# dusk-network/plonk

Measured on AMD Instinct MI355X. Metric: prove() wall-clock (ms) at 2^20 gates, lower is better.
Workload: dtype u32 limbs (Fr 256-bit / Fp 384-bit Montgomery)

## Files before the change

__graft_entry__.py:

```python
from __future__ import annotations

import concurrent.futures as cf
import os
import shutil
import subprocess
import sys

ROOT = os.path.dirname(os.path.abspath(__file__))
CSRC = os.path.join(ROOT, "plonk_amd", "csrc")
LIBDIR = os.path.join(ROOT, "plonk_amd", "lib")
OBJDIR = os.path.join(ROOT, "build", "obj")
LIB = os.path.join(LIBDIR, "libplonk_hip.so")
HIP_SOURCES = ["ntt.hip", "msm.hip", "msm_sort.hip", "capi.hip", "poly.hip", "prover.hip", "serial.hip", "comm.hip", "verify.hip", "diagnose.hip", "kzg.hip", "composer.hip", "msm_points.hip", "pairing.hip", "kzg_domain.hip"]
MSM_LARGE_BITS = os.environ.get("PLONK_BUILD_MSM_LARGE_BITS", "19")
MSM_MEDIUM = os.environ.get("PLONK_BUILD_MSM_MEDIUM", "") == "1"
HIP_VARIANTS = [("msm.hip", "nbl" + MSM_LARGE_BITS, ["-DPLONK_MSM_NB_BITS=" + MSM_LARGE_BITS]),
                ("msm_sort.hip", "nbl" + MSM_LARGE_BITS, ["-DPLONK_MSM_NB_BITS=" + MSM_LARGE_BITS])]
if MSM_MEDIUM:
    HIP_VARIANTS += [("msm.hip", "nbm17", ["-DPLONK_MSM_NB_BITS=17", "-DPLONK_MSM_WITH_MEDIUM"]),
                     ("msm_sort.hip", "nbm17", ["-DPLONK_MSM_NB_BITS=17", "-DPLONK_MSM_WITH_MEDIUM"])]
    HIP_FLAGS_EXTRA = ["-DPLONK_MSM_WITH_MEDIUM"]
else:
    HIP_FLAGS_EXTRA = []
HIPCC = shutil.which("hipcc") or "/opt/rocm/bin/hipcc"
# ... 65 lines not shown
        os.makedirs(os.path.dirname(DEV_ARITH_LIB), exist_ok=True)
        os.makedirs(OBJDIR, exist_ok=True)

        def compile_group(group: str) -> str:
            obj = os.path.join(OBJDIR, "dev_arith." + group + ".o")
            if _newer(obj, deps):
                subprocess.check_call([HIPCC, *HIP_FLAGS, "-DARITH_GROUP=ARITH_FAMILIES_" + group, "-c", src, "-o", obj])
            return obj

        with cf.ThreadPoolExecutor(max_workers=len(DEV_ARITH_GROUPS)) as ex:
            objs = list(ex.map(compile_group, DEV_ARITH_GROUPS))
        subprocess.check_call([HIPCC, "--offload-arch=gfx950", "-shared", "-fPIC", *objs, "-o", DEV_ARITH_LIB])
    if verbose:
        print(f"[build] {DEV_ARITH_LIB}")
    return DEV_ARITH_LIB


DEV_POLY_LIB = os.path.join(ROOT, "tests", "_build", "libdev_poly.so")


def build_dev_poly(verbose: bool = True) -> str:
    src = os.path.join(ROOT, "tests", "csrc", "dev_poly.hip")
    if not os.path.exists(src):
        return DEV_POLY_LIB
    if _newer(DEV_POLY_LIB, [src, LIB] + _headers()):
        os.makedirs(os.path.dirname(DEV_POLY_LIB), exist_ok=True)
        subprocess.check_call([HIPCC, *HIP_FLAGS, "-I" + CSRC, "-shared", src, "-o", DEV_POLY_LIB,
                               "-L" + LIBDIR, "-lplonk_hip", "-Wl,-rpath,$ORIGIN/../../plonk_amd/lib"])
    if verbose:
        print(f"[build] {DEV_POLY_LIB}")
    return DEV_POLY_LIB


DEV_MSM_SORT_LIB = os.path.join(ROOT, "tests", "_build", "libdev_msm_sort.so")


def build_dev_msm_sort(verbose: bool = True) -> str:
    src = os.path.join(ROOT, "tests", "csrc", "dev_msm_sort.hip")
    if not os.path.exists(src):
        return DEV_MSM_SORT_LIB
    if _newer(DEV_MSM_SORT_LIB, [src, LIB] + _headers()):
        os.makedirs(os.path.dirname(DEV_MSM_SORT_LIB), exist_ok=True)
        subprocess.check_call([HIPCC, *HIP_FLAGS, "-I" + CSRC, "-shared", src, "-o", DEV_MSM_SORT_LIB,
                               "-L" + LIBDIR, "-lplonk_hip", "-Wl,-rpath,$ORIGIN/../../plonk_amd/lib"])
    if verbose:
        print(f"[build] {DEV_MSM_SORT_LIB}")
    return DEV_MSM_SORT_LIB


DEV_KZG_DOMAIN_LIB = os.path.join(ROOT, "tests", "_build", "libdev_kzg_domain.so")


def build_dev_kzg_domain(verbose: bool = True) -> str:
    src = os.path.join(ROOT, "tests", "csrc", "dev_kzg_domain.hip")
    if not os.path.exists(src):
        return DEV_KZG_DOMAIN_LIB
    if _newer(DEV_KZG_DOMAIN_LIB, [src, LIB] + _headers()):
        os.makedirs(os.path.dirname(DEV_KZG_DOMAIN_LIB), exist_ok=True)
        subprocess.check_call([HIPCC, *HIP_FLAGS, "-I" + CSRC, "-shared", src, "-o", DEV_KZG_DOMAIN_LIB,
                               "-L" + LIBDIR, "-lplonk_hip", "-Wl,-rpath,$ORIGIN/../../plonk_amd/lib"])
    if verbose:
        print(f"[build] {DEV_KZG_DOMAIN_LIB}")
    return DEV_KZG_DOMAIN_LIB


def build() -> None:
    with cf.ThreadPoolExecutor(max_workers=1) as side:
        dev_arith = side.submit(build_dev_arith)
        build_hip()
        build_dev_poly()
        build_dev_msm_sort()
        build_dev_kzg_domain()
        build_oracle()
        build_fake_rccl()
        dev_arith.result()
    sys.path.insert(0, ROOT)
    import plonk_amd
    plonk_amd.load_library()


def smoke() -> None:
    sys.path.insert(0, ROOT)
    import random

    import plonk_amd
    from oracle import bls12_381 as E
    from oracle.fft import EvaluationDomain

    ctx = plonk_amd.Context(0)
    rnd = random.Random(7)
    L = 12
    coeffs = [rnd.randrange(E.Q) for _ in range((1 << 9) + 3)]
    got = ctx.ntt(coeffs, L, inverse=False, coset=True)
    assert got == EvaluationDomain(1 << L).coset_fft(coeffs), "NTT mismatch vs oracle"
    pts = [E.g1_mul(E.G1_GEN, rnd.randrange(1, E.Q)) for _ in range(64)]
    sc = [rnd.randrange(E.Q) for _ in range(64)]
    ctx.srs_load(pts)
    assert ctx.msm(sc) == E.msm_pippenger(pts, sc), "MSM mismatch vs oracle"
    print("smoke ok: NTT(2^12 coset) and MSM(64) bit-exact vs oracle")


if __name__ == "__main__":
    build()
# ... 1 lines not shown
```

plonk_amd/csrc/poly.hip:

```cpp
#include <cstdlib>

#include "plonk_internal.hpp"
#include "fr29.cuh"
#include "fp_safegcd.cuh"
#include "poly.hpp"

namespace plonk {

__device__ __forceinline__ Fr ldf(const Fr* p) {
  const uint4* q = reinterpret_cast<const uint4*>(p);
  uint4 a = q[0], b = q[1];
  Fr r;
  r.l[0] = a.x; r.l[1] = a.y; r.l[2] = a.z; r.l[3] = a.w;
  r.l[4] = b.x; r.l[5] = b.y; r.l[6] = b.z; r.l[7] = b.w;
  return r;
}
__device__ __forceinline__ void stf(Fr* p, const Fr& v) {
  uint4* q = reinterpret_cast<uint4*>(p);
  q[0] = make_uint4(v.l[0], v.l[1], v.l[2], v.l[3]);
  q[1] = make_uint4(v.l[4], v.l[5], v.l[6], v.l[7]);
}
__device__ __forceinline__ Fr small(uint32_t v, const Fr& one) {
  Fr acc = Fr::zero();
  Fr p = one;
  for (uint32_t b = v; b; b >>= 1) {
    if (b & 1) acc = acc + p;
    p = p.dbl();
  }
  return acc;
}

__global__ void fill_zero_kernel(Fr* p, uint64_t n) {
  const uint64_t i = (uint64_t)blockIdx.x * blockDim.x + threadIdx.x;
// ... 394 lines not shown
  HIP_TRY(hipGetLastError());
  return PLONK_OK;
}
int scan_prefix_product_apply(Ctx* c, Fr* data, uint64_t n, const Fr* totals, const Fr& carry_twiddle) {
  const uint32_t nb = scan_prefix_blocks(n);
  PScanArgs a{};
  a.one_t = tw_of(Fr::one());
  a.one_r = tw_plain(Fr::one());
  a.carry_t = tw_plain(carry_twiddle);
  a.has_carry = 1;
  pscan_launch_apply(c, nb, data, n, totals, a);
  HIP_TRY(hipGetLastError());
  return PLONK_OK;
}
int scan_suffix_sum(Ctx* c, Fr* data, uint64_t n, Fr* totals) { return scan_inplace<false, true>(c, data, n, totals); }

struct PermConst {
  Tw conv;
  Tw gamma_t;
  Tw bk_t[4];
  Tw b32_t;
  Tw one_t;
};
__device__ __forceinline__ Fr29 ld_slot(const void* base, uint64_t idx) {
  const uint4* q = reinterpret_cast<const uint4*>(reinterpret_cast<const Fr29Slot*>(base) + idx);
  const uint4 a = q[0], b = q[1];
  const uint32_t c = reinterpret_cast<const Fr29Slot*>(base)[idx].w[8];
  Fr29 r;
  r.l[0] = a.x; r.l[1] = a.y; r.l[2] = a.z; r.l[3] = a.w;
  r.l[4] = b.x; r.l[5] = b.y; r.l[6] = b.z; r.l[7] = b.w;
  r.l[8] = c;
  return r;
}
__global__ void __launch_bounds__(128) perm_terms_kernel(PermArgs a, PermConst k) {
  const uint64_t j0 = (uint64_t)blockIdx.x * blockDim.x + threadIdx.x;
  if (j0 >= a.count) return;
  const uint64_t i = a.first + j0;
  if (i == 0) {
    const Fr one = tw29(k.one_t).to_fr();
    stf(a.num, one);
    stf(a.den, one);
    return;
  }
  const uint64_t r = i - 1;
  Fr29 root = ld_slot(a.tw_lo29, r & ((1ull << a.lobits) - 1));
  if (a.use_hi) root = Fr29::mul(root, ld_slot(a.tw_hi29, r >> a.lobits));
  const Fr29 conv = tw29(k.conv), gamma_t = tw29(k.gamma_t), b32 = tw29(k.b32_t);
  Fr29 num, den;
#pragma unroll
  for (int j = 0; j < 4; ++j) {
    const Fr29 wg = Fr29::add_csub(Fr29::mul(ld29_(a.wires[j] + r), conv), gamma_t);
    const Fr29 nf = Fr29::add_csub(wg, Fr29::mul(root, tw29(k.bk_t[j])));
    const Fr29 df = Fr29::add_csub(wg, Fr29::mul(ld29_(a.sigma[j] + r), b32));
    num = j ? Fr29::mul(num, nf) : nf;
    den = j ? Fr29::mul(den, df) : df;
  }
  stf(a.num + i, num.to_fr());
  stf(a.den + i, den.to_fr());
}
__global__ void mul_arrays_kernel(Fr* __restrict__ a, const Fr* __restrict__ b, uint64_t n, int* zero_flag) {
  const uint64_t i = (uint64_t)blockIdx.x * blockDim.x + threadIdx.x;
  if (i >= n) return;
  const Fr y = ldf(b + i);
  if (zero_flag && y.is_zero()) *zero_flag = 1;
  stf(a + i, Fr29::mul(ld29_(a + i), Fr29::from_fr(y)).to_fr());
}

__device__ __forceinline__ Fr delta4(const Fr& f, const Fr& one) {
  const Fr two = one.dbl();
  return f * (f - one) * (f - two) * (f - two - one);
}

__device__ __forceinline__ Fr29 ld29(const Fr* p) { return Fr29::from_fr(ldf(p)); }
__device__ __forceinline__ Fr29 c29(const uint32_t (&v)[9]) {
  Fr29 r;
#pragma unroll
  for (int i = 0; i < 9; ++i) r.l[i] = v[i];
  return r;
}

struct WidgetConst {
  Tw conv, one_r, c1, c3, c9, c18, c81, c83, ed;
  Tw rg[4];
  Tw lg[5];
  Tw fx[4];
  Tw vr[3];
};
template <bool WIDGETS>
__global__ void __launch_bounds__(128, WIDGETS ? 2 : 4) quotient_kernel(QuotientArgs q, WidgetConst wc) {
  const uint64_t i = (uint64_t)blockIdx.x * blockDim.x + threadIdx.x;
  if (i >= q.n8) return;
// ... 223 lines not shown
  uint32_t nbits;
  uint64_t zero_at;
};
template <int E>
__global__ void __launch_bounds__(256) mul_powers_kernel(const Fr* __restrict__ src, Fr* __restrict__ dst, uint64_t n,
                                                         MulPowArgs a, uint64_t src_off, uint64_t exp_off) {
  const uint64_t g = (uint64_t)blockIdx.x * blockDim.x + threadIdx.x;
  if (g == 0 && a.zero_at != ~0ull) stf(dst + a.zero_at, Fr::zero());
  const uint64_t wave = g >> 6, lane = g & 63;
  const uint64_t first = wave * (64 * E) + lane;
  if (first >= n) return;
  const Fr29 add = Fr29::from_fr(a.addend);
  const uint64_t e = first + exp_off;
  Fr29 p = tw29(a.one_t);
  bool started = false;
#pragma unroll 1
  for (uint32_t b = 0; b < a.nbits; ++b) {
    if ((e >> b) & 1) {
      const Fr29 w = tw29(a.pw[b]);
      p = started ? Fr29::mul(p, w) : w;
      started = true;
    }
  }
  const Fr29 step = tw29(a.pw[6]);
#pragma unroll 1
  for (int k = 0; k < E; ++k) {
    const uint64_t i = first + 64ull * k;
    if (i >= n) break;
    stf(dst + i, Fr29::mul(Fr29::add_csub(ld29_(src + i + src_off), add), p).to_fr());
    if (E > 1) p = Fr29::mul(p, step);
  }
}

__global__ void fold_kernel(const Fr* __restrict__ src, Fr* __restrict__ dst, uint64_t n, uint32_t extra, Fr c) {
  const uint64_t i = (uint64_t)blockIdx.x * blockDim.x + threadIdx.x;
  if (i >= n) return;
  Fr v = ldf(src + i);
  if (i < extra) v = v + c * ldf(src + n + i);
  stf(dst + i, v);
}

__global__ void shard_pack_kernel(ShardPackArgs a) {
  const uint64_t i = (uint64_t)blockIdx.x * blockDim.x + threadIdx.x;
  const uint32_t k = blockIdx.y, peer = blockIdx.z;
  if (i >= a.stride) return;
  const Fr* F = a.F[k];
  Fr v = Fr::zero();
  if (i < a.per) {
    const uint64_t idx = (uint64_t)peer * a.per + i;
    if (idx < a.n) v = ldf(F + idx);
  } else {
    v = ldf(F + (i - a.per));
  }
  stf(a.send + ((uint64_t)peer * a.cpr + k) * a.stride + i, v);
}

__global__ void __launch_bounds__(128) shard_combine_kernel(ShardCombineArgs a) {
  const uint64_t i = (uint64_t)blockIdx.x * blockDim.x + threadIdx.x;
  if (i >= a.cnt + 8) return;
  const bool extra = i >= a.cnt;
  const uint64_t off = extra ? a.per + (i - a.cnt) : i;
  Fr F[8];
  for (uint32_t j = 0; j < a.Q; ++j)
    F[j] = ldf(a.recv + ((uint64_t)(j % a.W) * a.cpr + j / a.W) * a.stride + off);
  auto dft = [&](uint32_t i1) {
    Fr acc = Fr::zero();
// ... 68 lines not shown
  hipLaunchKernelGGL(gather_wires_kernel, grid, dim3(256), 0, c->stream, idx_dev, values, wires, constraints, n);
  HIP_TRY(hipGetLastError());
  return PLONK_OK;
}
int poly_scatter_pi(Ctx* c, Fr* dense, const uint64_t* idx, const Fr* val, uint64_t count) {
  if (!count) return PLONK_OK;
  hipLaunchKernelGGL(scatter_pi_kernel, grid1(count, 256), dim3(256), 0, c->stream, dense, idx, val, count);
  HIP_TRY(hipGetLastError());
  return PLONK_OK;
}
int poly_batch_inverse(Ctx* c, Fr* v, uint64_t n, bool twiddle_form) {
  static const BatchInvArgs a = [] {
    BatchInvArgs r;
    r.one_t = tw_of(Fr::one());
    r.one_r = tw_plain(Fr::one());
    r.conv = tw_of(Fr::from_u64(32));
    return r;
  }();
  const int cfg_env = c->cfg.bi_cfg;
  const int cfg = cfg_env >= 0 && cfg_env <= 3 ? cfg_env : (n <= (1ull << 17) ? 1 : 0);
#define BI_LAUNCH(T, E)                                                                                                              \
  do {                                                                                                                               \
    if (twiddle_form) hipLaunchKernelGGL((batch_inverse_kernel<true, T, E>), grid1(n, T * E), dim3(T), 0, c->stream, v, n, a);         \
    else hipLaunchKernelGGL((batch_inverse_kernel<false, T, E>), grid1(n, T * E), dim3(T), 0, c->stream, v, n, a);                     \
  } while (0)
  if (cfg == 1) BI_LAUNCH(64, 4);
  else if (cfg == 2) BI_LAUNCH(64, 16);
  else if (cfg == 3) BI_LAUNCH(128, 8);
  else BI_LAUNCH(256, 16);
#undef BI_LAUNCH
  HIP_TRY(hipGetLastError());
  return PLONK_OK;
}
int poly_perm_terms(Ctx* c, const PermArgs& a) {
  PermConst k;
  k.conv = tw_of(Fr::from_u64(32));
  k.gamma_t = tw_of(a.gamma);
  for (int j = 0; j < 4; ++j) k.bk_t[j] = tw_of(a.beta * a.ks[j]);
  k.b32_t = tw_of(a.beta * Fr::from_u64(32));
  k.one_t = tw_of(Fr::one());
  PermArgs r = a;
  if (r.count == 0) { r.first = 0; r.count = a.n; }
  if (r.first + r.count > a.n) return (plonk::set_last_error("invalid argument", __func__, __FILE__, __LINE__), PLONK_ERR_ARG);
  hipLaunchKernelGGL(perm_terms_kernel, grid1(r.count, 128), dim3(128), 0, c->stream, r, k);
  HIP_TRY(hipGetLastError());
  return PLONK_OK;
}
int poly_mul_arrays(Ctx* c, Fr* a, const Fr* b, uint64_t n, int* zero_flag) {
  hipLaunchKernelGGL(mul_arrays_kernel, grid1(n, 256), dim3(256), 0, c->stream, a, b, n, zero_flag);
  HIP_TRY(hipGetLastError());
  return PLONK_OK;
}
int poly_quotient(Ctx* c, const QuotientArgs& q) {
  prof_begin(c, 3);
  WidgetConst wc{};
  if (q.has[QS_RANGE] | q.has[QS_LOGIC] | q.has[QS_FIXED] | q.has[QS_VAR]) {
    wc.conv = tw_of(Fr::from_u64(32));
    wc.one_r = tw_plain(Fr::one());
    wc.c1 = tw_of(Fr::one()); wc.c3 = tw_of(Fr::from_u64(3)); wc.c9 = tw_of(Fr::from_u64(9));
    wc.c18 = tw_of(Fr::from_u64(18)); wc.c81 = tw_of(Fr::from_u64(81)); wc.c83 = tw_of(Fr::from_u64(83));
    wc.ed = tw_of(q.edwards_d);
    Fr k = q.range_ch.sqr(), w = q.range_ch;
    for (int j = 0; j < 4; ++j) { wc.rg[j] = tw_of(w); w = w * k; }
    k = q.logic_ch.sqr();
    const Fr lk[5] = {k.sqr() * k, Fr::one(), k, k.sqr(), k.sqr().sqr()};
    for (int j = 0; j < 5; ++j) wc.lg[j] = tw_of(lk[j] * q.logic_ch);
    k = q.fixed_ch.sqr(); w = q.fixed_ch;
    for (int j = 0; j < 4; ++j) { wc.fx[j] = tw_of(w); w = w * k; }
    k = q.var_ch.sqr(); w = q.var_ch;
    for (int j = 0; j < 3; ++j) { wc.vr[j] = tw_of(w); w = w * k; }
    hipLaunchKernelGGL(quotient_kernel<true>, grid1(q.n8, 128), dim3(128), 0, c->stream, q, wc);
  } else {
    hipLaunchKernelGGL(quotient_kernel<false>, grid1(q.n8, 128), dim3(128), 0, c->stream, q, wc);
// ... 48 lines not shown
  EvalArgsD d;
  Fr pts[EV_POINTS];
  int npts = 0;
  for (int k = 0; k < count; ++k) {
    d.items[k].poly = a.items[k].poly;
    d.items[k].len = a.items[k].len;
    int w = 0;
    while (w < npts && !(pts[w] == a.items[k].x)) ++w;
    if (w == npts) {
      if (npts == EV_POINTS) return (plonk::set_last_error("invalid argument", "poly_eval: more than 2 distinct points", __FILE__, __LINE__), PLONK_ERR_ARG);
      pts[npts++] = a.items[k].x;
      Fr29 p = Fr29::twiddle_from_fr(a.items[k].x);
      for (int b = 0; b < EV_PW; ++b) {
        for (int i = 0; i < 9; ++i) d.pw[w][b].w[i] = p.l[i];
        p = Fr29::mul(p, p);
      }
    }
    d.items[k].point = (uint32_t)w;
  }
  d.partial = a.partial;
  d.max_blocks = a.max_blocks;
  int levels = 0;
  while (levels < 8 && (1u << levels) < nb) ++levels;
  if (le == 2) {
    hipLaunchKernelGGL(eval_kernel<2>, dim3(nb, count), dim3(EV_T), 0, c->stream, d);
    hipLaunchKernelGGL(eval_final_kernel<2>, dim3(count), dim3(EV_T), 0, c->stream, d, nb, levels, out_dev);
  } else {
    hipLaunchKernelGGL(eval_kernel<4>, dim3(nb, count), dim3(EV_T), 0, c->stream, d);
    hipLaunchKernelGGL(eval_final_kernel<4>, dim3(count), dim3(EV_T), 0, c->stream, d, nb, levels, out_dev);
  }
  HIP_TRY(hipGetLastError());
  return PLONK_OK;
}
int poly_lincomb(Ctx* c, const LinCombArgs& a) {
  LinCombArgsD d;
  for (int k = 0; k < a.count; ++k) {
    d.t[k].p = a.t[k].p;
    d.t[k].len = a.t[k].len;
    d.t[k].st = tw_of(a.t[k].s);
  }
  d.count = a.count;
  d.len = a.len;
  d.constant = a.constant;
  d.out = a.out;
  hipLaunchKernelGGL(lincomb_kernel, grid1(a.len, 256), dim3(256), 0, c->stream, d);
  HIP_TRY(hipGetLastError());
  return PLONK_OK;
}
static void launch_mul_powers(Ctx* c, const Fr* src, Fr* dst, uint64_t n, const Fr& x, uint64_t src_off, uint64_t exp_off,
                              const Fr& addend = Fr::zero(), uint64_t zero_at = ~0ull) {
  if (!n) {
    if (zero_at != ~0ull) (void)poly_fill_zero(c, dst + zero_at, 1);
    return;
  }
  MulPowArgs a;
  const uint64_t emax = n - 1 + exp_off;
  uint32_t nbits = 7;
  while (nbits < MP_BITS && (emax >> nbits)) ++nbits;
  Fr29 p = Fr29::twiddle_from_fr(x);
  for (uint32_t b = 0; b < nbits; ++b) {
    for (int i = 0; i < 9; ++i) a.pw[b].w[i] = p.l[i];
    p = Fr29::mul(p, p);
  }
  a.one_t = tw_of(Fr::one());
  a.addend = addend;
  a.nbits = nbits;
  a.zero_at = zero_at;
  if (n <= (1ull << 17)) hipLaunchKernelGGL(mul_powers_kernel<1>, grid1(n, 256), dim3(256), 0, c->stream, src, dst, n, a, src_off, exp_off);
  else if (n <= (1ull << 19)) hipLaunchKernelGGL(mul_powers_kernel<4>, grid1((n + 3) / 4 + 64, 256), dim3(256), 0, c->stream, src, dst, n, a, src_off, exp_off);
  else hipLaunchKernelGGL(mul_powers_kernel<16>, grid1((n + 15) / 16 + 64, 256), dim3(256), 0, c->stream, src, dst, n, a, src_off, exp_off);
}
int poly_ruffini(Ctx* c, const Fr* src, Fr* dst, uint64_t len, const Fr& z, const Fr& zinv, Fr* scratch, Fr* totals) {
  launch_mul_powers(c, src, scratch, len, z, 0, 0);
  int rc = scan_suffix_sum(c, scratch, len, totals);
  if (rc) return rc;
  launch_mul_powers(c, scratch, dst, len - 1, zinv, 1, 1, Fr::zero(), len - 1);
  HIP_TRY(hipGetLastError());
  return PLONK_OK;
}

__device__ __forceinline__ void st_slot(void* base, uint64_t idx, const Fr29& v) {
  uint32_t* w = reinterpret_cast<Fr29Slot*>(base)[idx].w;
#pragma unroll
  for (int i = 0; i < 9; ++i) w[i] = v.l[i];
  w[9] = 0; w[10] = 0; w[11] = 0;
}
__global__ void __launch_bounds__(256) kzg_powers_kernel(void* __restrict__ tab, uint32_t count, Tw xt, Tw one_t) {
  const uint32_t i = blockIdx.x * blockDim.x + threadIdx.x;
  if (i >= count) return;
  st_slot(tab, i, pow_tw(tw29(xt), i, tw29(one_t)));
}
__global__ void __launch_bounds__(256) power_array_kernel(Fr* __restrict__ out, uint64_t n, Tw xt, Tw one_t) {
  const uint64_t i = (uint64_t)blockIdx.x * blockDim.x + threadIdx.x;
  if (i >= n) return;
  stf(out + i, Fr29::mul(Fr29::from_fr(Fr::one()), pow_tw(tw29(xt), i, tw29(one_t))).to_fr());
}
__global__ void __launch_bounds__(256) kzg_trim_kernel(KzgDesc* __restrict__ desc) {
  __shared__ unsigned long long best;
  const Fr* p = desc[blockIdx.x].p;
  uint64_t hi = desc[blockIdx.x].len;
  while (hi) {
    if (!threadIdx.x) best = 0;
    __syncthreads();
    const uint64_t lo = hi > 256 ? hi - 256 : 0, idx = lo + threadIdx.x;
    if (idx < hi && !ldf(p + idx).is_zero()) atomicMax(&best, (unsigned long long)(idx + 1));
    __syncthreads();
    const uint64_t b = best;
    __syncthreads();
    if (b) { hi = b; break; }
// ... 135 lines not shown
```

plonk_amd/csrc/poly.hpp:

```cpp
#pragma once
#include "plonk_internal.hpp"

namespace plonk {

enum { QS_M = 0, QS_L, QS_R, QS_O, QS_F, QS_C, QS_ARITH, QS_RANGE, QS_LOGIC, QS_FIXED, QS_VAR, QS_COUNT };

struct BlindArgs {
  int count;
  Fr b[3];
};
struct SplitArgs {
  Fr b[3];
  uint64_t len4;
};
struct PermArgs {
  uint64_t n;
  uint64_t first = 0, count = 0;
  const Fr* wires[4];
  const Fr* sigma[4];
  Fr beta, gamma;
  Fr ks[4];
  const void* tw_lo29;
  const void* tw_hi29;
  uint32_t lobits;
// ... 107 lines not shown

void prof_begin(Ctx* c, int slot);
void prof_end(Ctx* c, int slot);
void prof_host_add(Ctx* c, int slot, double ms);

int poly_fill_zero(Ctx* c, Fr* p, uint64_t n);
int poly_blind(Ctx* c, Fr* coeffs, uint64_t n, const BlindArgs& a);
int poly_split_t(Ctx* c, Fr* t, uint64_t n, uint64_t np, Fr* out, const SplitArgs& a);
int poly_trimmed_len(Ctx* c, const Fr* p, uint64_t n, unsigned long long* out_dev);
int poly_scatter_pi(Ctx* c, Fr* dense, const uint64_t* idx, const Fr* val, uint64_t count);
int poly_sigma_evals(Ctx* c, const uint32_t* map_dev, const Fr* roots, Fr* out, uint64_t n, uint64_t stride, const SigmaArgs& a);
int poly_gather_wires(Ctx* c, const uint32_t* idx_dev, const Fr* values, Fr* wires, uint64_t constraints, uint64_t n);
int poly_batch_inverse(Ctx* c, Fr* v, uint64_t n, bool twiddle_form = false);
int poly_perm_terms(Ctx* c, const PermArgs& a);
int poly_mul_arrays(Ctx* c, Fr* a, const Fr* b, uint64_t n, int* zero_flag);
int poly_quotient(Ctx* c, const QuotientArgs& q);
int poly_dealias(Ctx* c, Fr* t, uint64_t nq, const Fr low[7], const Fr& g_inv);
int poly_l1(Ctx* c, const Fr* linear, Fr* l1, uint64_t n8, const L1Args& a);
int poly_scale_array(Ctx* c, Fr* v, uint64_t n, const Fr& s);
int poly_from_mont(Ctx* c, const Fr* src, Fr* dst, uint64_t n);
void quotient_const(const Fr& c, int shift, uint32_t out[9]);
void quotient_data(const Fr& c, uint32_t out[9]);
int poly_eval(Ctx* c, EvalArgs& a, int count, uint64_t max_len, Fr* out_dev);
int poly_lincomb(Ctx* c, const LinCombArgs& a);
int poly_ruffini(Ctx* c, const Fr* src, Fr* dst, uint64_t len, const Fr& z, const Fr& zinv, Fr* scratch, Fr* totals);
static constexpr int SCAN_T = 256;
static constexpr int SCAN_MAXPER = 64;
static constexpr uint64_t SCAN_TOTALS = SCAN_T * SCAN_MAXPER + 1;
int scan_prefix_product(Ctx* c, Fr* data, uint64_t n, Fr* totals);
uint32_t scan_prefix_blocks(uint64_t n);
int scan_prefix_product_local(Ctx* c, Fr* data, uint64_t n, Fr* totals);
int scan_prefix_product_apply(Ctx* c, Fr* data, uint64_t n, const Fr* totals, const Fr& carry_twiddle);
int scan_suffix_sum(Ctx* c, Fr* data, uint64_t n, Fr* totals);

}
```

plonk_amd/csrc/prover.hip:

```cpp
#include <cstdlib>
#include <cstring>
#include <random>
#include <string>
#include <vector>

#include "poly.hpp"
#include "transcript.hpp"
#include <chrono>

#include "hostg1.hpp"
#include "finish_pool.hpp"
#include "widgets.hpp"
#include "permutation.hpp"
#include "diagnose.hpp"
#include "composer.hpp"

static_assert(plonk::DQ_M == plonk::QS_M && plonk::DQ_ARITH == plonk::QS_ARITH && plonk::DQ_VAR == plonk::QS_VAR &&
              plonk::DQ_COUNT == plonk::QS_COUNT, "diagnose_core.hpp selector ids");
static_assert(plonk::WQS_RANGE == plonk::QS_RANGE && plonk::WQS_LOGIC == plonk::QS_LOGIC && plonk::WQS_FIXED == plonk::QS_FIXED &&
              plonk::WQS_VAR == plonk::QS_VAR && plonk::WQS_COUNT == plonk::QS_COUNT, "widgets.hpp selector ids");

namespace plonk {

struct Prover {
// ... 990 lines not shown
      AccMark mark(c, (side_defer && k0 + kc == 4) ? p->ev_acc : nullptr);
      PTRY(msm_group(p, sc, ms, 4, 0, p->lag_table, p->lag_n, tl, sp, 1, k0, kc));
    }
    PTRY(msm_group(p, sc, ms, 4, 0, p->lag_table, p->lag_n, tl, sp, 2));
  } else {
    p->last_wire_launches = 1;
    AccMark mark(c, side_defer ? p->ev_acc : nullptr);
    const uint64_t ms[4] = {n + 2, n + 2, n + 2, n + 2};
    if (lag) {
      const Fr* sc[4] = {wires_dev, wires_dev + n, wires_dev + 2 * n, wires_dev + 3 * n};
      const Fr* tl[4] = {p->wscal, p->wscal + 2, p->wscal + 4, p->wscal + 6};
      const uint64_t sp[4] = {n, n, n, n};
      PTRY(msm_group(p, sc, ms, 4, 0, p->lag_table, p->lag_n, tl, sp));
    } else {
      const Fr* sc[4] = {p->wpoly, p->wpoly + np, p->wpoly + 2 * np, p->wpoly + 3 * np};
      PTRY(msm_group(p, sc, ms, 4, 0));
    }
  }
  if (side_defer) {
    SideScopeAfter side(c, p->ev_acc);
    PTRY(side_round1());
  }
  PTRY(absorb_commitments(p, tr, 0, 4, comm));

  Challenges ch;
  ch.beta = tr.challenge_scalar("beta");
  tr.append_scalar("beta", ch.beta);
  ch.gamma = tr.challenge_scalar("gamma");
  {
    prof_begin(c, 4);
    const PermArgs pa = perm_args(p, wires_dev, ch, tbn);
    gap.launching();
    HIP_TRY(hipMemsetAsync(p->flag_dev, 0, sizeof(int), c->stream));
    PTRY(poly_perm_terms(c, pa));
    PTRY(poly_batch_inverse(c, pa.den, n, true));
    PTRY(poly_mul_arrays(c, pa.num, pa.den, n, p->flag_dev));
    PTRY(scan_prefix_product(c, pa.num, n, p->totals));
    if (!z_from_evals) PTRY(blind_z(p, pa.num, bl, p->tmp8));
    prof_end(c, 4);
  }
  auto side_round2 = [&]() -> int {
    if (z_from_evals) {
      PTRY(blind_z(p, p->scratch, bl, p->tmp8b));
      HIP_TRY(hipMemcpyAsync(p->low_host + 28, p->zpoly, 7 * sizeof(Fr), hipMemcpyDeviceToHost, c->stream));
      HIP_TRY(hipEventRecord(p->ev_zlow, c->stream));
    }
    PTRY(ntt_device(c, p->zpoly, p->cos, p->tmp8b, L + p->lq, false, true, n + 3));
    HIP_TRY(hipEventRecord(p->ev_side, c->side_stream));
    return PLONK_OK;
  };
  if (z_from_evals) {
    HIP_TRY(hipMemcpyAsync(p->wscal + 8, bl + 8, 3 * sizeof(Fr), hipMemcpyHostToDevice, c->stream));
  } else {
    HIP_TRY(hipMemcpyAsync(p->low_host + 28, p->zpoly, 7 * sizeof(Fr), hipMemcpyDeviceToHost, c->stream));
    HIP_TRY(hipEventRecord(p->ev_zlow, c->stream));
  }
  if (!side_defer_z) {
    SideScope side(c, p->ev_ready);
    PTRY(side_round2());
  }
  {
    AccMark mark(c, side_defer_z ? p->ev_acc : nullptr);
    if (z_from_evals) {
      const Fr* sc[1] = {p->scratch};
      const Fr* tl[1] = {p->wscal + 8};
      const uint64_t ms[1] = {n + 3}, sp[1] = {n};
      PTRY(msm_group(p, sc, ms, 1, 4, p->lag_table, p->lag_n, tl, sp));
    } else {
      PTRY(msm_to(p, p->zpoly, n + 3, 4));
    }
// ... 53 lines not shown
    const uint64_t ms[4] = {n + 1, n + 1, n + 1, t4_len};
    PTRY(msm_group(p, sc, ms, 4, 5));
  }
  PTRY(absorb_commitments(p, tr, 5, 4, comm));
  if (*p->flag_host) return (plonk::set_last_error("invalid argument", __func__, __FILE__, __LINE__), PLONK_ERR_ARG);

  const Fr z_ch = tr.challenge_scalar("z_challenge");
  const Fr zw = z_ch * omega;
  Evals ev;
  {
    EvalArgs ea;
    const uint64_t max_len = eval_items(p, z_ch, zw, 0, np, &ea);
    gap.launching();
    PTRY(poly_eval(c, ea, 15, max_len, p->evout));
    HIP_TRY(hipMemcpyAsync(p->ev_host, p->evout, 15 * sizeof(Fr), hipMemcpyDeviceToHost, c->stream));
    const auto t_before = HostGap::clock::now();
    HIP_TRY(hipStreamSynchronize(c->stream));
    gap.synced(t_before);
    ev = unpack_evals(p->ev_host);
  }
  append_evaluations(tr, ev);

  const Fr v = tr.challenge_scalar("v_challenge");
  Opening op;
  PTRY(opening_point(p, z_ch, zw, &op));
  const Fr v_w = tr.challenge_scalar("v_w_challenge");
  {
    gap.launching();
    SideScope side(c, p->ev_ready);
    LinCombArgs la;
    wzw_terms(p, v_w, 0, np, &la);
    la.len = np - 1;
    la.constant = Fr::zero();
    la.out = p->tmp8;
    PTRY(poly_lincomb(c, la));
    PTRY(poly_ruffini(c, p->tmp8, p->wit2, np - 1, zw, op.inv_z * p->omega_inv, p->scratch + np, p->totals2));
    HIP_TRY(hipEventRecord(p->ev_side, c->side_stream));
  }
  opening_scalars(p, ev, ch, z_ch, v, pi_idx, pi_val, pi_count, &op);
  {
    LinCombArgs la;
    numerator_terms(p, ev, ch, op, t4, t4_len, 0, np, &la);
    la.len = np - 1;
    la.constant = op.pi_eval;
    la.out = p->agg;
    gap.launching();
    PTRY(poly_lincomb(c, la));
  }
  PTRY(poly_ruffini(c, p->agg, p->wit, np - 1, z_ch, op.inv_z, p->scratch, p->totals));
  HIP_TRY(hipMemcpyAsync(p->evout + 15, p->scratch, sizeof(Fr), hipMemcpyDeviceToDevice, c->stream));
  HIP_TRY(hipMemcpyAsync(p->ev_host + 15, p->evout + 15, sizeof(Fr), hipMemcpyDeviceToHost, c->stream));
  HIP_TRY(hipStreamWaitEvent(c->main_stream, p->ev_side, 0));
  {
    const Fr* sc[2] = {p->wit, p->wit2};
    const uint64_t ms[2] = {np - 2, np - 2};
    PTRY(msm_group(p, sc, ms, 2, 9));
  }
  PTRY(fetch_commitments(p, 9, 2, comm + 9));
  if (!quotient_identity_holds(p->ev_host[15], ev, ch.alpha, ch.beta, ch.gamma, op.l1_z, op.vp)) return PLONK_ERR_UNSAT;

  write_proof(proof, comm, ev);
  return PLONK_OK;
}

static int prover_prove_sharded(Prover* p, const Fr* wires_dev, const uint64_t* pi_idx, const Fr* pi_val, uint64_t pi_count,
                                const Fr* bl, uint8_t proof[1008]) {
  Ctx* c = p->c;
  if (p->srs_gen != c->srs_gen) return (set_last_error("prover is bound to an SRS that was replaced on its context", __func__, __FILE__, __LINE__), PLONK_ERR_STATE);
  const uint64_t n = p->n, np = p->np, qn = p->qn;
  const uint32_t L = p->logn, W = (uint32_t)p->world, cpr = p->cpr, Q = p->Q;
  const uint64_t lo = p->lo, hi = p->hi;
  NttTables* tbn;
  PTRY(ntt_tables(c, L, false, &tbn));
  const Fr omega = p->omega;

  Transcript tr((const uint8_t*)p->label.data(), p->label.size());
  seed_transcript(tr, p, pi_val, pi_count);
  HostGap gap{c};
  GapScope gap_scope(&gap);

  uint8_t comm[11][48];
  const bool lag = p->lag_on;
// ... 869 lines not shown
```

Before: 31.30.

## Fuse permutation grand product and lincomb+Ruffini into blockwise scan kernels

```diff
diff --git a/__graft_entry__.py b/__graft_entry__.py
--- a/__graft_entry__.py
+++ b/__graft_entry__.py
@@ -121,6 +121,22 @@
     return DEV_POLY_LIB
 
 
+DEV_POLY_FUSED_LIB = os.path.join(ROOT, "tests", "_build", "libdev_poly_fused.so")
+
+
+def build_dev_poly_fused(verbose: bool = True) -> str:
+    src = os.path.join(ROOT, "tests", "csrc", "dev_poly_fused.hip")
+    if not os.path.exists(src):
+        return DEV_POLY_FUSED_LIB
+    if _newer(DEV_POLY_FUSED_LIB, [src, LIB] + _headers()):
+        os.makedirs(os.path.dirname(DEV_POLY_FUSED_LIB), exist_ok=True)
+        subprocess.check_call([HIPCC, *HIP_FLAGS, "-I" + CSRC, "-shared", src, "-o", DEV_POLY_FUSED_LIB,
+                               "-L" + LIBDIR, "-lplonk_hip", "-Wl,-rpath,$ORIGIN/../../plonk_amd/lib"])
+    if verbose:
+        print(f"[build] {DEV_POLY_FUSED_LIB}")
+    return DEV_POLY_FUSED_LIB
+
+
 DEV_MSM_SORT_LIB = os.path.join(ROOT, "tests", "_build", "libdev_msm_sort.so")
 
 
@@ -158,6 +174,7 @@
         dev_arith = side.submit(build_dev_arith)
         build_hip()
         build_dev_poly()
+        build_dev_poly_fused()
         build_dev_msm_sort()
         build_dev_kzg_domain()
         build_oracle()
diff --git a/plonk_amd/csrc/poly.hip b/plonk_amd/csrc/poly.hip
--- a/plonk_amd/csrc/poly.hip
+++ b/plonk_amd/csrc/poly.hip
@@ -1,4 +1,5 @@
 #include <cstdlib>
+#include <type_traits>
 
 #include "plonk_internal.hpp"
 #include "fr29.cuh"
@@ -459,6 +460,22 @@
   r.l[8] = c;
   return r;
 }
+__device__ __forceinline__ void perm_row(const PermArgs& a, const PermConst& k, uint64_t r, Fr29* num_out, Fr29* den_out) {
+  Fr29 root = ld_slot(a.tw_lo29, r & ((1ull << a.lobits) - 1));
+  if (a.use_hi) root = Fr29::mul(root, ld_slot(a.tw_hi29, r >> a.lobits));
+  const Fr29 conv = tw29(k.conv), gamma_t = tw29(k.gamma_t), b32 = tw29(k.b32_t);
+  Fr29 num, den;
+#pragma unroll
+  for (int j = 0; j < 4; ++j) {
+    const Fr29 wg = Fr29::add_csub(Fr29::mul(ld29_(a.wires[j] + r), conv), gamma_t);
+    const Fr29 nf = Fr29::add_csub(wg, Fr29::mul(root, tw29(k.bk_t[j])));
+    const Fr29 df = Fr29::add_csub(wg, Fr29::mul(ld29_(a.sigma[j] + r), b32));
+    num = j ? Fr29::mul(num, nf) : nf;
+    den = j ? Fr29::mul(den, df) : df;
+  }
+  *num_out = num;
+  *den_out = den;
+}
 __global__ void __launch_bounds__(128) perm_terms_kernel(PermArgs a, PermConst k) {
   const uint64_t j0 = (uint64_t)blockIdx.x * blockDim.x + threadIdx.x;
   if (j0 >= a.count) return;
@@ -469,21 +486,130 @@
     stf(a.den, one);
     return;
   }
-  const uint64_t r = i - 1;
-  Fr29 root = ld_slot(a.tw_lo29, r & ((1ull << a.lobits) - 1));
-  if (a.use_hi) root = Fr29::mul(root, ld_slot(a.tw_hi29, r >> a.lobits));
-  const Fr29 conv = tw29(k.conv), gamma_t = tw29(k.gamma_t), b32 = tw29(k.b32_t);
   Fr29 num, den;
-#pragma unroll
-  for (int j = 0; j < 4; ++j) {
-    const Fr29 wg = Fr29::add_csub(Fr29::mul(ld29_(a.wires[j] + r), conv), gamma_t);
-    const Fr29 nf = Fr29::add_csub(wg, Fr29::mul(root, tw29(k.bk_t[j])));
-    const Fr29 df = Fr29::add_csub(wg, Fr29::mul(ld29_(a.sigma[j] + r), b32));
-    num = j ? Fr29::mul(num, nf) : nf;
-    den = j ? Fr29::mul(den, df) : df;
-  }
+  perm_row(a, k, i - 1, &num, &den);
   stf(a.num + i, num.to_fr());
   stf(a.den + i, den.to_fr());
+}
+
+__device__ __forceinline__ bool is_zero29(const Fr29& x) {
+  const Fr29 c = x.csub_q();
+  uint32_t any = 0;
+#pragma unroll
+  for (int i = 0; i < 9; ++i) any |= c.l[i];
+  return any == 0;
+}
+__device__ __forceinline__ void ps_lanes_both(Fr29& p, Fr29& s, uint32_t (*shp)[SCAN_T], uint32_t (*shs)[SCAN_T], int t,
+                                              const Fr29& one_t, Fr29* ptot, Fr29* stot) {
+  for (int d = 1; d < SCAN_T; d <<= 1) {
+    ps_put(shp, t, p);
+    ps_put(shs, t, s);
+    __syncthreads();
+    if (t >= d) p = Fr29::mul(ps_get(shp, t - d), p);
+    if (t + d < SCAN_T) s = Fr29::mul(ps_get(shs, t + d), s);
+    __syncthreads();
+  }
+  ps_put(shp, t, p);
+  ps_put(shs, t, s);
+  __syncthreads();
+  p = t ? ps_get(shp, t - 1) : one_t;
+  s = (t + 1 < SCAN_T) ? ps_get(shs, t + 1) : one_t;
+  *ptot = ps_get(shp, SCAN_T - 1);
+  *stot = ps_get(shs, 0);
+}
+template <int I, int N, class F>
+__device__ __forceinline__ void unrolled(F&& f) {
+  if constexpr (I < N) {
+    f(std::integral_constant<int, I>{});
+    unrolled<I + 1, N>(f);
+  }
+}
+template <int E>
+__global__ void __launch_bounds__(SCAN_T) gp_block_kernel(PermArgs a, PermConst k, Fr* __restrict__ totals, uint32_t nb, int* flag) {
+  __shared__ uint32_t shp[9][SCAN_T], shs[9][SCAN_T];
+  const int t = threadIdx.x;
+  const uint64_t base = (uint64_t)blockIdx.x * (SCAN_T * E) + (uint64_t)t * E;
+  const Fr29 one_t = tw29(k.one_t);
+  Fr29 v[E], d[E];
+  Fr29 accn = one_t, accd = one_t;
+  unrolled<0, E>([&](auto ec) {
+    constexpr int e = decltype(ec)::value;
+    const uint64_t i = base + e;
+    d[e] = one_t;
+    if (i > 0 && i < a.n) {
+      Fr29 num, den;
+      perm_row(a, k, i - 1, &num, &den);
+      if (is_zero29(den)) *flag = 1;
+      else d[e] = den;
+      accn = Fr29::mul(accn, num);
+      accd = Fr29::mul(accd, d[e]);
+    }
+    v[e] = accn;
+  });
+  Fr29 ntot, dtot;
+  ps_lanes_both(accn, accd, shp, shs, t, one_t, &ntot, &dtot);
+  if (t == 0) {
+    stf(totals + blockIdx.x, ntot.to_fr());
+    stf(totals + nb + blockIdx.x, dtot.to_fr());
+  }
+  unrolled<0, E>([&](auto ec) {
+    constexpr int e = E - 1 - decltype(ec)::value;
+    const uint64_t i = base + e;
+    if (i < a.n) {
+      stf(a.num + i, Fr29::mul(accn, v[e]).to_fr());
+      stf(a.den + i, accd.to_fr());
+    }
+    accd = Fr29::mul(accd, d[e]);
+  });
+}
+__global__ void __launch_bounds__(SCAN_T) gp_totals_kernel(Fr* __restrict__ totals, uint32_t nb, uint32_t per, PScanArgs a) {
+  __shared__ uint32_t shp[9][SCAN_T], shs[9][SCAN_T], shinv[9];
+  const int t = threadIdx.x;
+  Fr* const tn = totals;
+  const Fr* const td = totals + nb;
+  const Fr29 one_t = tw29(a.one_t);
+  Fr29 accn = one_t, accd = one_t;
+  for (uint32_t j = 0; j < per; ++j) {
+    const uint32_t i = t * per + j;
+    if (i < nb) {
+      accn = Fr29::mul(accn, ld29_(tn + i));
+      accd = Fr29::mul(accd, ld29_(td + i));
+    }
+  }
+  Fr29 ntot, dtot;
+  ps_lanes_both(accn, accd, shp, shs, t, one_t, &ntot, &dtot);
+  if (t == 0) {
+    const Fr29 r = fr29_inv_gcd_tw(dtot);
+#pragma unroll
+    for (int i = 0; i < 9; ++i) shinv[i] = r.l[i];
+  }
+  __syncthreads();
+  Fr29 inv;
+#pragma unroll
+  for (int i = 0; i < 9; ++i) inv.l[i] = shinv[i];
+  for (uint32_t j = 0; j < per; ++j) {
+    const uint32_t i = t * per + j;
+    if (i < nb) {
+      const Fr29 x = ld29_(tn + i);
+      stf(tn + i, accn.to_fr());
+      accn = Fr29::mul(accn, x);
+    }
+  }
+  accd = Fr29::mul(Fr29::mul(accd, inv), tw29(a.one_r));
+  for (uint32_t j = per; j-- > 0;) {
+    const uint32_t i = t * per + j;
+    if (i < nb) {
+      stf(tn + i, Fr29::mul(ld29_(tn + i), accd).to_fr());
+      accd = Fr29::mul(accd, ld29_(td + i));
+    }
+  }
+}
+__global__ void __launch_bounds__(256) gp_apply_kernel(const Fr* a, const Fr* b, Fr* z, uint64_t n, const Fr* __restrict__ totals,
+                                                       uint32_t block_log) {
+  const uint64_t i = (uint64_t)blockIdx.x * blockDim.x + threadIdx.x;
+  if (i >= n) return;
+  const Fr29 c = ld29_(totals + (i >> block_log));
+  stf(z + i, Fr29::mul(Fr29::mul(ld29_(a + i), ld29_(b + i)), c).to_fr());
 }
 __global__ void mul_arrays_kernel(Fr* __restrict__ a, const Fr* __restrict__ b, uint64_t n, int* zero_flag) {
   const uint64_t i = (uint64_t)blockIdx.x * blockDim.x + threadIdx.x;
@@ -773,6 +899,111 @@
   }
 }
 
+static inline int lrscan_e(uint64_t len) { return len <= (1ull << 17) ? 2 : 4; }
+template <int E>
+__global__ void __launch_bounds__(SCAN_T) lincomb_ruffini_block_kernel(LinCombArgsD a, MulPowArgs m, Fr* __restrict__ scratch,
+                                                                       Fr* __restrict__ totals, uint32_t nb) {
+  __shared__ Fr sh[SCAN_T];
+  const int t = threadIdx.x;
+  const uint64_t base = (uint64_t)blockIdx.x * (SCAN_T * E) + (uint64_t)t * E;
+  Fr29 p = tw29(m.one_t);
+  if (base < a.len) {
+    bool started = false;
+#pragma unroll 1
+    for (uint32_t b = 0; b < m.nbits; ++b) {
+      if ((base >> b) & 1) {
+        const Fr29 w = tw29(m.pw[b]);
+        p = started ? Fr29::mul(p, w) : w;
+        started = true;
+      }
+    }
+  }
+  const Fr29 step = tw29(m.pw[0]);
+  Fr29 c[E];
+  unrolled<0, E>([&](auto ec) {
+    constexpr int e = decltype(ec)::value;
+    c[e] = (base + e == 0) ? Fr29::from_fr(a.constant) : Fr29::zero();
+  });
+  for (int k = 0; k < a.count; ++k) {
+    const Fr* const tp = a.t[k].p;
+    const uint64_t tl = a.t[k].len;
+    const Fr29 st = tw29(a.t[k].st);
+    unrolled<0, E>([&](auto ec) {
+      constexpr int e = decltype(ec)::value;
+      if (base + e < tl) c[e] = Fr29::add_csub(c[e], Fr29::mul(ld29_(tp + base + e), st));
+    });
+  }
+  Fr v[E];
+  unrolled<0, E>([&](auto ec) {
+    constexpr int e = decltype(ec)::value;
+    v[e] = Fr::zero();
+    if (base + e < a.len) {
+      v[e] = Fr29::mul(c[e], p).to_fr();
+      p = Fr29::mul(p, step);
+    }
+  });
+  Fr acc = Fr::zero();
+  unrolled<0, E>([&](auto ec) {
+    constexpr int e = E - 1 - decltype(ec)::value;
+    acc = acc + v[e];
+    v[e] = acc;
+  });
+  sh[t] = acc;
+  __syncthreads();
+  for (int d = 1; d < SCAN_T; d <<= 1) {
+    Fr x = Fr::zero();
+    const bool take = t + d < SCAN_T;
+    if (take) x = sh[t + d];
+    __syncthreads();
+    if (take) sh[t] = sh[t] + x;
+    __syncthreads();
+  }
+  const Fr excl = (t + 1 < SCAN_T) ? sh[t + 1] : Fr::zero();
+  if (t == 0) stf(totals + (nb - 1 - blockIdx.x), sh[0]);
+  unrolled<0, E>([&](auto ec) {
+    constexpr int e = decltype(ec)::value;
+    if (base + e < a.len) stf(scratch + base + e, excl + v[e]);
+  });
+}
+template <int E>
+__global__ void __launch_bounds__(256) ruffini_apply_kernel(Fr* __restrict__ scratch, Fr* __restrict__ dst, uint64_t n, MulPowArgs a,
+                                                            const Fr* __restrict__ totals, uint32_t nb, uint32_t block_log) {
+  const uint64_t g = (uint64_t)blockIdx.x * blockDim.x + threadIdx.x;
+  if (g == 0) {
+    stf(dst + n, Fr::zero());
+    if (nb > 1) stf(scratch, ldf(scratch) + ldf(totals + nb - 2));
+  }
+  const uint64_t wave = g >> 6, lane = g & 63;
+  const uint64_t first = wave * (64 * E) + lane;
+  if (first >= n) return;
+  const uint64_t e = first + 1;
+  Fr29 p = tw29(a.one_t);
+  bool started = false;
+#pragma unroll 1
+  for (uint32_t b = 0; b < a.nbits; ++b) {
+    if ((e >> b) & 1) {
+      const Fr29 w = tw29(a.pw[b]);
+      p = started ? Fr29::mul(p, w) : w;
+      started = true;
+    }
+  }
+  const Fr29 step = tw29(a.pw[6]);
+  uint64_t cur = ~0ull;
+  Fr off = Fr::zero();
+#pragma unroll 1
+  for (int k = 0; k < E; ++k) {
+    const uint64_t i = first + 64ull * k;
+    if (i >= n) break;
+    const uint64_t b = (i + 1) >> block_log;
+    if (b != cur) {
+      cur = b;
+      off = (b + 1 < nb) ? ldf(totals + (nb - 2 - b)) : Fr::zero();
+    }
+    stf(dst + i, Fr29::mul(Fr29::from_fr(ldf(scratch + i + 1) + off), p).to_fr());
+    if (E > 1) p = Fr29::mul(p, step);
+  }
+}
+
 __global__ void fold_kernel(const Fr* __restrict__ src, Fr* __restrict__ dst, uint64_t n, uint32_t extra, Fr c) {
   const uint64_t i = (uint64_t)blockIdx.x * blockDim.x + threadIdx.x;
   if (i >= n) return;
@@ -907,13 +1138,34 @@
   HIP_TRY(hipGetLastError());
   return PLONK_OK;
 }
-int poly_perm_terms(Ctx* c, const PermArgs& a) {
+static PermConst perm_const(const PermArgs& a) {
   PermConst k;
   k.conv = tw_of(Fr::from_u64(32));
   k.gamma_t = tw_of(a.gamma);
   for (int j = 0; j < 4; ++j) k.bk_t[j] = tw_of(a.beta * a.ks[j]);
   k.b32_t = tw_of(a.beta * Fr::from_u64(32));
   k.one_t = tw_of(Fr::one());
+  return k;
+}
+int poly_grand_product(Ctx* c, const PermArgs& a, Fr* z, Fr* totals, int* flag) {
+  const uint64_t n = a.n;
+  const uint32_t nb = scan_prefix_blocks(n);
+  if (n == 0 || a.first != 0 || (a.count != 0 && a.count != n) || 2ull * nb > SCAN_TOTALS || nb > (uint32_t)SCAN_T * SCAN_MAXPER)
+    return (plonk::set_last_error("invalid argument", __func__, __FILE__, __LINE__), PLONK_ERR_ARG);
+  const PermConst k = perm_const(a);
+  PScanArgs s{};
+  s.one_t = tw_of(Fr::one());
+  s.one_r = tw_plain(Fr::one());
+  const int e = pscan_e(n);
+  if (e == 2) hipLaunchKernelGGL(gp_block_kernel<2>, dim3(nb), dim3(SCAN_T), 0, c->stream, a, k, totals, nb, flag);
+  else hipLaunchKernelGGL(gp_block_kernel<8>, dim3(nb), dim3(SCAN_T), 0, c->stream, a, k, totals, nb, flag);
+  hipLaunchKernelGGL(gp_totals_kernel, dim3(1), dim3(SCAN_T), 0, c->stream, totals, nb, (nb + SCAN_T - 1) / SCAN_T, s);
+  hipLaunchKernelGGL(gp_apply_kernel, grid1(n, 256), dim3(256), 0, c->stream, a.num, a.den, z, n, totals, e == 2 ? 9u : 11u);
+  HIP_TRY(hipGetLastError());
+  return PLONK_OK;
+}
+int poly_perm_terms(Ctx* c, const PermArgs& a) {
+  const PermConst k = perm_const(a);
   PermArgs r = a;
   if (r.count == 0) { r.first = 0; r.count = a.n; }
   if (r.first + r.count > a.n) return (plonk::set_last_error("invalid argument", __func__, __FILE__, __LINE__), PLONK_ERR_ARG);
@@ -1028,7 +1280,7 @@
   HIP_TRY(hipGetLastError());
   return PLONK_OK;
 }
-int poly_lincomb(Ctx* c, const LinCombArgs& a) {
+static LinCombArgsD lincomb_dev(const LinCombArgs& a) {
   LinCombArgsD d;
   for (int k = 0; k < a.count; ++k) {
     d.t[k].p = a.t[k].p;
@@ -1039,18 +1291,16 @@
   d.len = a.len;
   d.constant = a.constant;
   d.out = a.out;
+  return d;
+}
+int poly_lincomb(Ctx* c, const LinCombArgs& a) {
+  const LinCombArgsD d = lincomb_dev(a);
   hipLaunchKernelGGL(lincomb_kernel, grid1(a.len, 256), dim3(256), 0, c->stream, d);
   HIP_TRY(hipGetLastError());
   return PLONK_OK;
 }
-static void launch_mul_powers(Ctx* c, const Fr* src, Fr* dst, uint64_t n, const Fr& x, uint64_t src_off, uint64_t exp_off,
-                              const Fr& addend = Fr::zero(), uint64_t zero_at = ~0ull) {
-  if (!n) {
-    if (zero_at != ~0ull) (void)poly_fill_zero(c, dst + zero_at, 1);
-    return;
-  }
+static MulPowArgs mul_pow_args(const Fr& x, uint64_t emax) {
   MulPowArgs a;
-  const uint64_t emax = n - 1 + exp_off;
   uint32_t nbits = 7;
   while (nbits < MP_BITS && (emax >> nbits)) ++nbits;
   Fr29 p = Fr29::twiddle_from_fr(x);
@@ -1059,8 +1309,19 @@
     p = Fr29::mul(p, p);
   }
   a.one_t = tw_of(Fr::one());
+  a.addend = Fr::zero();
+  a.nbits = nbits;
+  a.zero_at = ~0ull;
+  return a;
+}
+static void launch_mul_powers(Ctx* c, const Fr* src, Fr* dst, uint64_t n, const Fr& x, uint64_t src_off, uint64_t exp_off,
+                              const Fr& addend = Fr::zero(), uint64_t zero_at = ~0ull) {
+  if (!n) {
+    if (zero_at != ~0ull) (void)poly_fill_zero(c, dst + zero_at, 1);
+    return;
+  }
+  MulPowArgs a = mul_pow_args(x, n - 1 + exp_off);
   a.addend = addend;
-  a.nbits = nbits;
   a.zero_at = zero_at;
   if (n <= (1ull << 17)) hipLaunchKernelGGL(mul_powers_kernel<1>, grid1(n, 256), dim3(256), 0, c->stream, src, dst, n, a, src_off, exp_off);
   else if (n <= (1ull << 19)) hipLaunchKernelGGL(mul_powers_kernel<4>, grid1((n + 3) / 4 + 64, 256), dim3(256), 0, c->stream, src, dst, n, a, src_off, exp_off);
@@ -1071,6 +1332,27 @@
   int rc = scan_suffix_sum(c, scratch, len, totals);
   if (rc) return rc;
   launch_mul_powers(c, scratch, dst, len - 1, zinv, 1, 1, Fr::zero(), len - 1);
+  HIP_TRY(hipGetLastError());
+  return PLONK_OK;
+}
+int poly_lincomb_ruffini(Ctx* c, const LinCombArgs& a, Fr* dst, const Fr& z, const Fr& zinv, Fr* scratch, Fr* totals) {
+  const uint64_t len = a.len;
+  const int e = lrscan_e(len);
+  const uint32_t block_log = e == 2 ? 9 : 10;
+  const uint64_t nb64 = (len + (1ull << block_log) - 1) >> block_log;
+  if (len == 0 || a.count < 0 || a.count > 24 || nb64 > (uint64_t)SCAN_T * SCAN_MAXPER)
+    return (plonk::set_last_error("invalid argument", __func__, __FILE__, __LINE__), PLONK_ERR_ARG);
+  const uint32_t nb = (uint32_t)nb64;
+  const LinCombArgsD d = lincomb_dev(a);
+  const MulPowArgs mz = mul_pow_args(z, len - 1);
+  if (e == 2) hipLaunchKernelGGL(lincomb_ruffini_block_kernel<2>, dim3(nb), dim3(SCAN_T), 0, c->stream, d, mz, scratch, totals, nb);
+  else hipLaunchKernelGGL(lincomb_ruffini_block_kernel<4>, dim3(nb), dim3(SCAN_T), 0, c->stream, d, mz, scratch, totals, nb);
+  if (nb > 1) hipLaunchKernelGGL((scan_totals_kernel<false>), dim3(1), dim3(SCAN_T), 0, c->stream, totals, nb, (nb + SCAN_T - 1) / SCAN_T);
+  const uint64_t n = len - 1;
+  const MulPowArgs mi = mul_pow_args(zinv, len);
+  if (n <= (1ull << 17)) hipLaunchKernelGGL(ruffini_apply_kernel<1>, grid1(n ? n : 1, 256), dim3(256), 0, c->stream, scratch, dst, n, mi, totals, nb, block_log);
+  else if (n <= (1ull << 19)) hipLaunchKernelGGL(ruffini_apply_kernel<4>, grid1((n + 3) / 4 + 64, 256), dim3(256), 0, c->stream, scratch, dst, n, mi, totals, nb, block_log);
+  else hipLaunchKernelGGL(ruffini_apply_kernel<16>, grid1((n + 15) / 16 + 64, 256), dim3(256), 0, c->stream, scratch, dst, n, mi, totals, nb, block_log);
   HIP_TRY(hipGetLastError());
   return PLONK_OK;
 }
diff --git a/plonk_amd/csrc/poly.hpp b/plonk_amd/csrc/poly.hpp
--- a/plonk_amd/csrc/poly.hpp
+++ b/plonk_amd/csrc/poly.hpp
@@ -163,5 +163,7 @@
 int scan_prefix_product_local(Ctx* c, Fr* data, uint64_t n, Fr* totals);
 int scan_prefix_product_apply(Ctx* c, Fr* data, uint64_t n, const Fr* totals, const Fr& carry_twiddle);
 int scan_suffix_sum(Ctx* c, Fr* data, uint64_t n, Fr* totals);
+int poly_grand_product(Ctx* c, const PermArgs& a, Fr* z, Fr* totals, int* flag);
+int poly_lincomb_ruffini(Ctx* c, const LinCombArgs& a, Fr* dst, const Fr& z, const Fr& zinv, Fr* scratch, Fr* totals);
 
 }
diff --git a/plonk_amd/csrc/prover.hip b/plonk_amd/csrc/prover.hip
--- a/plonk_amd/csrc/prover.hip
+++ b/plonk_amd/csrc/prover.hip
@@ -1046,10 +1046,14 @@
     const PermArgs pa = perm_args(p, wires_dev, ch, tbn);
     gap.launching();
     HIP_TRY(hipMemsetAsync(p->flag_dev, 0, sizeof(int), c->stream));
-    PTRY(poly_perm_terms(c, pa));
-    PTRY(poly_batch_inverse(c, pa.den, n, true));
-    PTRY(poly_mul_arrays(c, pa.num, pa.den, n, p->flag_dev));
-    PTRY(scan_prefix_product(c, pa.num, n, p->totals));
+    if (2ull * scan_prefix_blocks(n) <= SCAN_TOTALS) {
+      PTRY(poly_grand_product(c, pa, pa.num, p->totals, p->flag_dev));
+    } else {
+      PTRY(poly_perm_terms(c, pa));
+      PTRY(poly_batch_inverse(c, pa.den, n, true));
+      PTRY(poly_mul_arrays(c, pa.num, pa.den, n, p->flag_dev));
+      PTRY(scan_prefix_product(c, pa.num, n, p->totals));
+    }
     if (!z_from_evals) PTRY(blind_z(p, pa.num, bl, p->tmp8));
     prof_end(c, 4);
   }
@@ -1169,9 +1173,8 @@
     wzw_terms(p, v_w, 0, np, &la);
     la.len = np - 1;
     la.constant = Fr::zero();
-    la.out = p->tmp8;
-    PTRY(poly_lincomb(c, la));
-    PTRY(poly_ruffini(c, p->tmp8, p->wit2, np - 1, zw, op.inv_z * p->omega_inv, p->scratch + np, p->totals2));
+    la.out = nullptr;
+    PTRY(poly_lincomb_ruffini(c, la, p->wit2, zw, op.inv_z * p->omega_inv, p->scratch + np, p->totals2));
     HIP_TRY(hipEventRecord(p->ev_side, c->side_stream));
   }
   opening_scalars(p, ev, ch, z_ch, v, pi_idx, pi_val, pi_count, &op);
@@ -1180,11 +1183,10 @@
     numerator_terms(p, ev, ch, op, t4, t4_len, 0, np, &la);
     la.len = np - 1;
     la.constant = op.pi_eval;
-    la.out = p->agg;
+    la.out = nullptr;
     gap.launching();
-    PTRY(poly_lincomb(c, la));
-  }
-  PTRY(poly_ruffini(c, p->agg, p->wit, np - 1, z_ch, op.inv_z, p->scratch, p->totals));
+    PTRY(poly_lincomb_ruffini(c, la, p->wit, z_ch, op.inv_z, p->scratch, p->totals));
+  }
   HIP_TRY(hipMemcpyAsync(p->evout + 15, p->scratch, sizeof(Fr), hipMemcpyDeviceToDevice, c->stream));
   HIP_TRY(hipMemcpyAsync(p->ev_host + 15, p->evout + 15, sizeof(Fr), hipMemcpyDeviceToHost, c->stream));
   HIP_TRY(hipStreamWaitEvent(c->main_stream, p->ev_side, 0));
```

New measurement: 31.24, median of 4. About the same (-0.2%).
